# Boese0601/MagicDance

Measured on NVIDIA H100. Metric: denoise-steps/sec @512x512 50-step DDIM, higher is better.
Workload: dtype f16

## Files before the change

### magicdance_b200/csrc/attention.cu

```cuda
#include <stdlib.h>

#include <type_traits>

#include "common.cuh"

namespace mdb {

constexpr int kBQ = 128;

template <int D, int BKV, int STAGES>
struct AttnCfg {
  static constexpr int kDkChunks = (D + 63) / 64;
  static constexpr int kDV = (D + 15) / 16 * 16;
  static constexpr int kKSteps = kDV / 16;
  static constexpr int kQBytes = kDkChunks * kBQ * 128;
  static constexpr int kKBytes = kDkChunks * BKV * 128;
  static constexpr int kVBytes = kDV * 128;
  static constexpr int kStageBytes = kKBytes + kVBytes;
  static constexpr int kSmem = kQBytes + STAGES * kStageBytes + 1024;
  static_assert(BKV == 64, "one 128-byte swizzle row of keys per V^T tile");
  static_assert(kVBytes % 1024 == 0 && kKBytes % 1024 == 0, "stage tiles start on swizzle-atom boundaries");
};

struct AttnKParams {
  CUtensorMap tmQ, tmK0, tmV0, tmK1, tmV1;
  __half* out;
  long long ldo;
  int nq, n0, n1;
  int kv0_batches, kv1_batches;
  int ldv0_batch, ldv1_batch;
  int bank_batches;
  float scale_log2;
};
struct AttnLseKParams : AttnKParams {
  float* lse;
};

template <int D, int BKV, int STAGES, int MINB, bool LSE = false>
__global__ void __launch_bounds__(kWsThreads, MINB)
    attn_wg_kernel(const __grid_constant__ std::conditional_t<LSE, AttnLseKParams, AttnKParams> p) {
  using C = AttnCfg<D, BKV, STAGES>;
  extern __shared__ uint8_t smem_raw[];
  __shared__ __align__(8) uint64_t q_bar;
  __shared__ __align__(8) uint64_t kv_full[STAGES], kv_empty[STAGES];

  uint8_t* sQ = align1024(smem_raw);
  uint8_t* sKV = sQ + C::kQBytes;

  const int warp = threadIdx.x >> 5;
  const int lane = threadIdx.x & 31;
  const int q0 = blockIdx.x * kBQ;
  const int head = blockIdx.y;
  const int b = blockIdx.z;
  const int t0 = (p.n0 + BKV - 1) / BKV;
  const int t1 = (b < p.bank_batches && p.n1 > 0) ? (p.n1 + BKV - 1) / BKV : 0;
  const int n_tiles = t0 + t1;

  pdl_launch_dependents();
  if (warp == kProducerWarp && lane == 0) {
    tma_prefetch_desc(&p.tmQ);
    tma_prefetch_desc(&p.tmK0);
    tma_prefetch_desc(&p.tmV0);
    mbar_init(&q_bar, 1);
    ring_init<STAGES>(kv_full, kv_empty, 1);
    fence_barrier_init();
  }
  __syncthreads();
  pdl_wait();

  if (warp == kProducerWarp) {
    if (lane == 0) {
      mbar_expect_tx(&q_bar, C::kQBytes);
      for (int dc = 0; dc < C::kDkChunks; ++dc)
        tma_load_3d(sQ + dc * (kBQ * 128), &p.tmQ, &q_bar, dc * 64, head, b * p.nq + q0);
      for (int j = 0; j < n_tiles; ++j) {
        const bool src1 = j >= t0;
        const int key0 = (src1 ? (j - t0) : j) * BKV;
        const CUtensorMap* tk = src1 ? &p.tmK1 : &p.tmK0;
        const CUtensorMap* tv = src1 ? &p.tmV1 : &p.tmV0;
        const int nsrc = src1 ? p.n1 : p.n0;
        const int kvb = src1 ? (p.kv1_batches > 1 ? b : 0) : (p.kv0_batches > 1 ? b : 0);
        const int ldvb = src1 ? p.ldv1_batch : p.ldv0_batch;
        const int s = ring_acquire<STAGES>(kv_empty, j);
        mbar_expect_tx(&kv_full[s], C::kStageBytes);
        uint8_t* sk = sKV + s * C::kStageBytes;
        uint8_t* sv = sk + C::kKBytes;
        for (int dc = 0; dc < C::kDkChunks; ++dc)
          tma_load_3d(sk + dc * (BKV * 128), tk, &kv_full[s], dc * 64, head, kvb * nsrc + key0);
        tma_load_2d(sv, tv, &kv_full[s], kvb * ldvb + key0, head * D);
      }
    }
  } else {
    const int wg = warp >> 2;
    const uint32_t q_addr = smem_u32(sQ) + wg * (64 * 128);
    const int cq = 2 * (lane & 3);
    float o[C::kDV / 2];
#pragma unroll
    for (int i = 0; i < C::kDV / 2; ++i) o[i] = 0.f;
    float m_run[2] = {-INFINITY, -INFINITY};
    float l_run[2] = {0.f, 0.f};
    mbar_wait(&q_bar, 0);

    for (int j = 0; j < n_tiles; ++j) {
      const bool src1 = j >= t0;
      const int key0 = (src1 ? (j - t0) : j) * BKV;
      const int valid = min(BKV, (src1 ? p.n1 : p.n0) - key0);
      const int s = ring_wait_full<STAGES>(kv_full, j);
      const uint32_t k_addr = smem_u32(sKV + s * C::kStageBytes);
      const uint32_t v_addr = k_addr + C::kKBytes;

      float sc[BKV / 2];
      wgmma_fence();
#pragma unroll
      for (int ks = 0; ks < C::kKSteps; ++ks) {
        const int dc = ks >> 2, kk = ks & 3;
        const uint64_t da = wgmma_desc_k_sw128(q_addr + dc * (kBQ * 128)) + 2 * kk;
        const uint64_t db = wgmma_desc_k_sw128(k_addr + dc * (BKV * 128)) + 2 * kk;
        wgmma_ss<BKV>(sc, da, db, ks != 0 ? 1u : 0u);
      }
      wgmma_commit();
      wgmma_wait<0>();
      wgmma_fence_regs(sc);

      if (valid < BKV) {
#pragma unroll
        for (int i = 0; i < BKV / 2; ++i)
          if (8 * (i >> 2) + cq + (i & 1) >= valid) sc[i] = -INFINITY;
      }
      float mx[2] = {-INFINITY, -INFINITY};
#pragma unroll
      for (int i = 0; i < BKV / 2; ++i) mx[(i >> 1) & 1] = fmaxf(mx[(i >> 1) & 1], sc[i]);
      float alpha[2], neg_m[2];
#pragma unroll
      for (int h = 0; h < 2; ++h) {
        mx[h] = fmaxf(mx[h], __shfl_xor_sync(0xffffffffu, mx[h], 1));
        mx[h] = fmaxf(mx[h], __shfl_xor_sync(0xffffffffu, mx[h], 2));
        const float m_new = fmaxf(m_run[h], mx[h] * p.scale_log2);
        alpha[h] = ex2_approx(m_run[h] - m_new);
        m_run[h] = m_new;
        neg_m[h] = -m_new;
      }
      float ls[2] = {0.f, 0.f};
      uint32_t pa[BKV / 16][4];
#pragma unroll
      for (int i = 0; i < BKV / 2; i += 2) {
        const int h = (i >> 1) & 1;
        const float e0 = ex2_approx(fmaf(sc[i], p.scale_log2, neg_m[h]));
        const float e1 = ex2_approx(fmaf(sc[i + 1], p.scale_log2, neg_m[h]));
        ls[h] += e0 + e1;
        pa[i >> 3][(i >> 1) & 3] = pack_half2(e0, e1);
      }
#pragma unroll
      for (int h = 0; h < 2; ++h) l_run[h] = fmaf(l_run[h], alpha[h], ls[h]);
#pragma unroll
      for (int i = 0; i < C::kDV / 2; ++i) o[i] *= alpha[(i >> 1) & 1];

      wgmma_fence();
#pragma unroll
      for (int kk = 0; kk < BKV / 16; ++kk)
        wgmma_rs<C::kDV>(o, pa[kk], wgmma_desc_k_sw128(v_addr) + 2 * kk, 1u);
      wgmma_commit();
      wgmma_wait<0>();
      wgmma_fence_regs(o);
      mbar_arrive(&kv_empty[s]);
    }

    float inv_l[2], l_row[2];
#pragma unroll
    for (int h = 0; h < 2; ++h) {
      float l = l_run[h];
      l += __shfl_xor_sync(0xffffffffu, l, 1);
      l += __shfl_xor_sync(0xffffffffu, l, 2);
      inv_l[h] = 1.0f / l;
      l_row[h] = l;
    }
    const int r = wg * 64 + (warp & 3) * 16 + (lane >> 2);
    if constexpr (LSE) {
      if ((lane & 3) == 0) {
#pragma unroll
        for (int h = 0; h < 2; ++h) {
          const int q = q0 + r + 8 * h;
          if (q < p.nq)
            p.lse[(static_cast<long long>(b) * gridDim.y + head) * p.nq + q] =
                (m_run[h] + log2f(l_row[h])) * 0.6931471805599453f;
        }
      }
    }
#pragma unroll
    for (int h = 0; h < 2; ++h) {
      const int q = q0 + r + 8 * h;
      if (q < p.nq) {
        __half* op = p.out + (static_cast<long long>(b) * p.nq + q) * p.ldo + head * D + cq;
#pragma unroll
        for (int c8 = 0; c8 < D / 8; ++c8)
          *reinterpret_cast<uint32_t*>(op + 8 * c8) =
              pack_half2(o[4 * c8 + 2 * h] * inv_l[h], o[4 * c8 + 2 * h + 1] * inv_l[h]);
      }
    }
  }
}

static int g_attn40_2q_min_ctas = 512;
int get_attn_tuning() { return g_attn40_2q_min_ctas; }
void set_attn_tuning(int v) { g_attn40_2q_min_ctas = v; }

template <int D, int BKV, int STAGES, int MINB, bool LSE = false, typename P>
static int launch_attn(const P& kp, dim3 grid, cudaStream_t st) {
  using C = AttnCfg<D, BKV, STAGES>;
  static_assert(MINB == 1 || C::kSmem <= 113 * 1024, "two CTAs per SM must fit");
  constexpr auto kern = attn_wg_kernel<D, BKV, STAGES, MINB, LSE>;
  if (int rc = set_max_dyn_smem<kern>(C::kSmem)) return rc;
  MDB_CHECK_CUDA(launch_pdl(kern, grid, dim3(kWsThreads), C::kSmem, st, kp));
  count_launch();
  return MDB_OK;
}

template <int D, int BKV>
static int build_and_launch(const mdb_attn_desc* a, float* lse, cudaStream_t st) {
  constexpr int kDV = AttnCfg<D, BKV, 1>::kDV;
  AttnKParams kp;
  memset(&kp, 0, sizeof(kp));
  const int hd = a->heads * a->d;
  int rc;
  if ((rc = tmap_heads(&kp.tmQ, a->q, a->d, a->heads, (uint64_t)a->batch * a->nq, a->ldq, kBQ))) return rc;
  auto mk_kv = [&](const void* k, long long ldk, const void* vt, long long ldvt, int n, int nb, int ldvb,
                   CUtensorMap* tk, CUtensorMap* tv) -> int {
    int r = tmap_heads(tk, k, a->d, a->heads, (uint64_t)nb * n, ldk, BKV);
    if (r) return r;
    return tmap_rows(tv, vt, (uint64_t)nb * ldvb, hd, ldvt, 64, kDV);
  };
  if ((rc = mk_kv(a->k0, a->ldk0, a->vt0, a->ldvt0, a->n0, a->kv0_batches, a->ldv0_batch, &kp.tmK0, &kp.tmV0))) return rc;
  if (a->n1 > 0) {
    if ((rc = mk_kv(a->k1, a->ldk1, a->vt1, a->ldvt1, a->n1, a->kv1_batches, a->ldv1_batch, &kp.tmK1, &kp.tmV1)))
      return rc;
  }
  kp.out = static_cast<__half*>(a->out);
  kp.ldo = a->ldo;
  kp.nq = a->nq;
  kp.n0 = a->n0;
  kp.n1 = a->n1;
  kp.kv0_batches = a->kv0_batches;
  kp.kv1_batches = a->kv1_batches;
  kp.ldv0_batch = a->ldv0_batch;
  kp.ldv1_batch = a->ldv1_batch;
  kp.bank_batches = a->n1 > 0 ? a->bank_batches : 0;
  kp.scale_log2 = a->scale * 1.4426950408889634f;
  dim3 grid((a->nq + kBQ - 1) / kBQ, a->heads, a->batch);
  if (lse != nullptr) {
    AttnLseKParams lp;
    memset(&lp, 0, sizeof(lp));
    static_cast<AttnKParams&>(lp) = kp;
    lp.lse = lse;
    if constexpr (D == 40) {
      const long long ctas = (long long)grid.x * grid.y * grid.z;
      if (ctas >= (long long)g_attn40_2q_min_ctas) return launch_attn<D, BKV, 3, 2, true>(lp, grid, st);
    }
    return launch_attn<D, BKV, (D == 160 ? 2 : 4), 1, true>(lp, grid, st);
  }
  if constexpr (D == 40) {
    const long long ctas = (long long)grid.x * grid.y * grid.z;
    if (ctas >= (long long)g_attn40_2q_min_ctas) return launch_attn<D, BKV, 3, 2>(kp, grid, st);
  }
// ... 48 lines not shown
```

### magicdance_b200/csrc/common.cuh

```cuda
#pragma once

#include <cuda.h>
#include <cuda_fp16.h>
#include <cuda_runtime.h>
#include <cudaTypedefs.h>
#include <stdint.h>
#include <stdio.h>
#include <string.h>

#include "../../include/magicdance_b200.h"
#include "wgmma.cuh"

namespace mdb {

void set_error(const char* fmt, ...);

#define MDB_CHECK_CUDA(expr)                                                                     \
  do {                                                                                           \
    cudaError_t _e = (expr);                                                                     \
    if (_e != cudaSuccess) {                                                                     \
      mdb::set_error("%s:%d: %s failed: %s", __FILE__, __LINE__, #expr, cudaGetErrorString(_e)); \
      return MDB_ERR_CUDA;                                                                       \
    }                                                                                            \
  } while (0)

#define MDB_REQUIRE(cond, ...)      \
  do {                              \
    if (!(cond)) {                  \
      mdb::set_error(__VA_ARGS__);  \
      return MDB_ERR_INVALID;       \
    }                               \
  } while (0)

void count_launch(int n = 1);
int get_gemm_tuning(int key);
void set_gemm_tuning(int key, int value);
int get_attn_tuning();
void set_attn_tuning(int v);

constexpr int kNumSms = 132;

int tmap_rows(CUtensorMap* out, const void* base, uint64_t inner, uint64_t rows, long long ld, uint32_t box_inner,
              uint32_t box_rows);
int tmap_heads(CUtensorMap* out, const void* base, int d, int heads, uint64_t tokens, long long ld,
               uint32_t box_tokens);
int tmap_nhwc(CUtensorMap* out, const void* base, int c, int w, int h, int nb, long long ld, const uint32_t box[4],
              int cs);

enum { kBoxOk, kBoxWideRows, kBoxRowsPerTile, kBoxImagesPerTile, kBoxTooLarge };
int pixel_box(int ho, int wo, int cs, int rows, bool fwd, uint32_t box[4]);

#ifdef __CUDACC__

bool pdl_enabled();
template <typename... KArgs, typename... Args>
inline cudaError_t launch_pdl_cluster2(void (*kernel)(KArgs...), dim3 grid, dim3 block, size_t smem,
                                       cudaStream_t stream, unsigned cluster_x, unsigned cluster_z, Args&&... args) {
  cudaLaunchConfig_t cfg;
  memset(&cfg, 0, sizeof(cfg));
  cfg.gridDim = grid;
  cfg.blockDim = block;
  cfg.dynamicSmemBytes = smem;
  cfg.stream = stream;
  cudaLaunchAttribute attr[2];
  int n = 0;
  if (cluster_z > 1 || cluster_x > 1) {
    attr[n].id = cudaLaunchAttributeClusterDimension;
    attr[n].val.clusterDim.x = cluster_x;
    attr[n].val.clusterDim.y = 1;
    attr[n].val.clusterDim.z = cluster_z;
    ++n;
  }
  if (pdl_enabled()) {
    attr[n].id = cudaLaunchAttributeProgrammaticStreamSerialization;
    attr[n].val.programmaticStreamSerializationAllowed = 1;
    ++n;
// ... 44 lines not shown
}
__device__ __forceinline__ void fence_barrier_init() {
  asm volatile("fence.mbarrier_init.release.cluster;" ::: "memory");
}
__device__ __forceinline__ void mbar_expect_tx(uint64_t* bar, uint32_t bytes) {
  asm volatile("mbarrier.arrive.expect_tx.shared::cta.b64 _, [%0], %1;" ::"r"(smem_u32(bar)), "r"(bytes)
               : "memory");
}
__device__ __forceinline__ void mbar_arrive(uint64_t* bar) {
  asm volatile("mbarrier.arrive.shared::cta.b64 _, [%0];" ::"r"(smem_u32(bar)) : "memory");
}
__device__ __forceinline__ void mbar_wait(uint64_t* bar, uint32_t parity) {
  uint32_t addr = smem_u32(bar);
  asm volatile(
      "{\n\t.reg .pred P1;\n\t"
      "WAIT_LOOP:\n\t"
      "mbarrier.try_wait.parity.shared::cta.b64 P1, [%0], %1;\n\t"
      "@P1 bra DONE;\n\t"
      "bra WAIT_LOOP;\n\t"
      "DONE:\n\t}"
      ::"r"(addr), "r"(parity)
      : "memory");
}

constexpr int kConsumers = 256;
constexpr int kProducerWarp = kConsumers / 32;
constexpr int kWsThreads = kConsumers + 32;

__device__ __forceinline__ uint8_t* align1024(uint8_t* p) {
  return reinterpret_cast<uint8_t*>((reinterpret_cast<uintptr_t>(p) + 1023) & ~uintptr_t(1023));
}

template <int S>
__device__ __forceinline__ void ring_init(uint64_t* full, uint64_t* empty, uint32_t full_count) {
  for (int s = 0; s < S; ++s) {
    mbar_init(&full[s], full_count);
    mbar_init(&empty[s], kConsumers);
  }
}
template <int S>
__device__ __forceinline__ int ring_acquire(uint64_t* empty, int it) {
  const int s = it % S;
  mbar_wait(&empty[s], ((it / S) & 1) ^ 1);
  return s;
}
template <int S>
__device__ __forceinline__ int ring_wait_full(uint64_t* full, int it) {
  const int s = it % S;
  mbar_wait(&full[s], (it / S) & 1);
  return s;
}

__device__ __forceinline__ void tma_prefetch_desc(const CUtensorMap* m) {
  asm volatile("prefetch.tensormap [%0];" ::"l"(reinterpret_cast<uint64_t>(m)) : "memory");
}
__device__ __forceinline__ void tma_load_2d(void* dst, const CUtensorMap* m, uint64_t* bar, int c0, int c1) {
  asm volatile(
      "cp.async.bulk.tensor.2d.shared::cluster.global.tile.mbarrier::complete_tx::bytes [%0], [%1, {%3, %4}], [%2];"
      ::"r"(smem_u32(dst)), "l"(reinterpret_cast<uint64_t>(m)), "r"(smem_u32(bar)), "r"(c0), "r"(c1)
      : "memory");
}
__device__ __forceinline__ void tma_load_3d(void* dst, const CUtensorMap* m, uint64_t* bar, int c0, int c1, int c2) {
  asm volatile(
      "cp.async.bulk.tensor.3d.shared::cluster.global.tile.mbarrier::complete_tx::bytes [%0], [%1, {%3, %4, %5}], [%2];"
      ::"r"(smem_u32(dst)), "l"(reinterpret_cast<uint64_t>(m)), "r"(smem_u32(bar)), "r"(c0), "r"(c1), "r"(c2)
      : "memory");
}
__device__ __forceinline__ void tma_load_4d(void* dst, const CUtensorMap* m, uint64_t* bar, int c0, int c1, int c2,
                                            int c3) {
  asm volatile(
// ... 76 lines not shown
```

### magicdance_b200/csrc/gemm.cu

```cuda
#include <stdlib.h>

#include "common.cuh"

namespace mdb {

constexpr int kBM = 128;
constexpr int kBK = 64;

struct GemmKParams {
  CUtensorMap tmA;
  CUtensorMap tmA2;
  CUtensorMap tmB;
  __half* d;
  long long ldd;
  const float* bias;
  long long bias_batch_stride;
  const __half* residual;
  long long ldr;
  float* ws;
  int rows_per_batch;
  int m, n;
  int k_chunks;
  int k1_chunks;
  int chunks_per_split;
  int splits;
  int conv;
  int chunks_per_tap;
  int w, hw;
  int cs;
  int cluster_reduce;
  const float* ln_u;
  float ln_eps;
};

template <int BN, int STAGES>
struct GemmSmem {
  static constexpr int kABytes = kBM * kBK * 2;
  static constexpr int kBBytes = BN * kBK * 2;
  static constexpr int kStageBytes = kABytes + kBBytes;
  static constexpr int kTotal = STAGES * kStageBytes + 1024;
  static constexpr int kCtasPerSm = (kTotal <= 113 * 1024 && BN <= 128) ? 2 : 1;
};

__device__ __forceinline__ void epi_store_chunk(const GemmKParams& p, long long row, int col0, int ncols,
                                                float (&v)[32], const float* bias_chunk) {
  const __half* rp = (p.residual != nullptr) ? p.residual + row * p.ldr + col0 : nullptr;
  __half* dp = p.d + row * p.ldd + col0;
#pragma unroll
  for (int q = 0; q < 4; ++q) {
    if (q * 8 + 8 <= ncols) {
      float o[8];
#pragma unroll
      for (int e = 0; e < 8; ++e) o[e] = v[q * 8 + e];
      if (bias_chunk != nullptr) {
        const float4 b0 = *reinterpret_cast<const float4*>(bias_chunk + q * 8);
        const float4 b1 = *reinterpret_cast<const float4*>(bias_chunk + q * 8 + 4);
        o[0] += b0.x; o[1] += b0.y; o[2] += b0.z; o[3] += b0.w;
        o[4] += b1.x; o[5] += b1.y; o[6] += b1.z; o[7] += b1.w;
      }
      if (rp != nullptr) {
        const uint4 r4 = *reinterpret_cast<const uint4*>(rp + q * 8);
        const __half2* h2 = reinterpret_cast<const __half2*>(&r4);
#pragma unroll
        for (int e = 0; e < 4; ++e) {
          const float2 f = __half22float2(h2[e]);
          o[2 * e] += f.x;
          o[2 * e + 1] += f.y;
        }
      }
      uint4 o4;
      o4.x = pack_half2(o[0], o[1]);
      o4.y = pack_half2(o[2], o[3]);
      o4.z = pack_half2(o[4], o[5]);
      o4.w = pack_half2(o[6], o[7]);
      *reinterpret_cast<uint4*>(dp + q * 8) = o4;
    } else if (q * 8 < ncols) {
// ... 24 lines not shown

  uint8_t* smem = align1024(smem_raw);
  const int warp = threadIdx.x >> 5;
  const int lane = threadIdx.x & 31;
  const int m0 = blockIdx.x * kBM;
  const int n0 = blockIdx.y * BN;
  const int split = blockIdx.z;
  const int kc_begin = split * p.chunks_per_split;
  const int kc_end = min(p.k_chunks, kc_begin + p.chunks_per_split);
  const int n_iter = kc_end - kc_begin;
  constexpr int kRedLd = BN + 4;
  static_assert(kBM * kRedLd * 4 <= kStages * S::kStageBytes, "the accumulator tile must fit in the operand ring");
  const bool ln = p.ln_u != nullptr;

  pdl_launch_dependents();
  if (warp == kProducerWarp && lane == 0) {
    tma_prefetch_desc(&p.tmA);
    tma_prefetch_desc(&p.tmB);
    ring_init<kStages>(full_bar, empty_bar, 1);
    fence_barrier_init();
  }
  const bool bias_in_smem = (p.bias != nullptr) && (p.bias_batch_stride == 0) && !p.cluster_reduce;
  if (bias_in_smem && warp < kProducerWarp) {
    for (int j = threadIdx.x; j < BN; j += kConsumers) s_bias[j] = (n0 + j < p.n) ? p.bias[n0 + j] : 0.f;
  }
  if (ln && warp < kProducerWarp) {
    for (int j = threadIdx.x; j < BN; j += kConsumers) s_lnu[j] = (n0 + j < p.n) ? p.ln_u[n0 + j] : 0.f;
  }
  __syncthreads();
  pdl_wait();

  if (warp == kProducerWarp) {
    if (lane == 0 && n_iter > 0) {
      int b0 = 0, y0 = 0, x0 = 0;
      if (p.conv) {
        b0 = m0 / p.hw;
        y0 = (p.hw >= kBM) ? (m0 % p.hw) / p.w : 0;
        x0 = (p.hw >= kBM) ? (m0 % p.hw) % p.w : 0;
      }
      for (int it = 0; it < n_iter; ++it) {
        const int s = ring_acquire<kStages>(empty_bar, it);
        uint8_t* sa = smem + s * S::kStageBytes;
        uint8_t* sb = sa + S::kABytes;
        const int kc = kc_begin + it;
        mbar_expect_tx(&full_bar[s], S::kStageBytes);
        if (p.conv) {
          const int tap = kc / p.chunks_per_tap;
          const int cc = kc - tap * p.chunks_per_tap;
          const int kh = tap / 3, kw = tap - kh * 3;
          tma_load_4d(sa, &p.tmA, &full_bar[s], cc * kBK, p.cs * x0 + kw - 1, p.cs * y0 + kh - 1, b0);
        } else if (kc < p.k1_chunks) {
          tma_load_2d(sa, &p.tmA, &full_bar[s], kc * kBK, m0);
        } else {
          tma_load_2d(sa, &p.tmA2, &full_bar[s], (kc - p.k1_chunks) * kBK, m0);
        }
        tma_load_2d(sb, &p.tmB, &full_bar[s], kc * kBK, n0);
      }
    }
  } else {
    const int wg = warp >> 2;
    const int tid = threadIdx.x;
    float acc[BN / 2];
#pragma unroll
    for (int i = 0; i < BN / 2; ++i) acc[i] = 0.f;
    const int ln_row = tid >> 1, ln_half = tid & 1;
    float pivot = 0.f, ls0 = 0.f, ls1 = 0.f, lq0 = 0.f, lq1 = 0.f;
    for (int it = 0; it < n_iter; ++it) {
      const int s = ring_wait_full<kStages>(full_bar, it);
      const uint32_t a_addr = smem_u32(smem + s * S::kStageBytes);
      const uint64_t da = wgmma_desc_k_sw128(a_addr + wg * (64 * 128));
      const uint64_t db = wgmma_desc_k_sw128(a_addr + S::kABytes);
      wgmma_fence();
#pragma unroll
      for (int k = 0; k < kBK / 16; ++k) wgmma_ss<BN>(acc, da + 2 * k, db + 2 * k, 1u);
      wgmma_commit();
      if (ln) {
        const uint32_t arow = a_addr + (ln_row >> 3) * 1024 + (ln_row & 7) * 128;
        if (it == 0) {
          uint32_t w0;
          asm volatile("ld.shared.b32 %0, [%1];" : "=r"(w0) : "r"(arow + ((0 ^ (ln_row & 7)) << 4)));
          pivot = __low2float(*reinterpret_cast<const __half2*>(&w0));
        }
#pragma unroll
        for (int l = ln_half * 4; l < ln_half * 4 + 4; ++l) {
          uint4 u4;
          asm volatile("ld.shared.v4.b32 {%0, %1, %2, %3}, [%4];"
                       : "=r"(u4.x), "=r"(u4.y), "=r"(u4.z), "=r"(u4.w)
                       : "r"(arow + ((l ^ (ln_row & 7)) << 4)));
          const __half2* h2 = reinterpret_cast<const __half2*>(&u4);
// ... 227 lines not shown
      }
      if (p.bias != nullptr) {
        const long long brow = (p.bias_batch_stride != 0) ? (row / p.rows_per_batch) : 0;
        const float* bp = p.bias + brow * p.bias_batch_stride + col;
        a.x += bp[0]; a.y += bp[1]; a.z += bp[2]; a.w += bp[3];
      }
      if (p.residual != nullptr) {
        const __half2* rp = reinterpret_cast<const __half2*>(p.residual + row * p.ldr + col);
        const float2 r0 = __half22float2(rp[0]), r1 = __half22float2(rp[1]);
        a.x += r0.x; a.y += r0.y; a.z += r1.x; a.w += r1.y;
      }
      uint2 o;
      o.x = pack_half2(a.x, a.y);
      o.y = pack_half2(a.z, a.w);
      *reinterpret_cast<uint2*>(p.d + row * p.ldd + col) = o;
    }
    return;
  }
  for (long long i = static_cast<long long>(blockIdx.x) * blockDim.x + threadIdx.x; i < slab;
       i += static_cast<long long>(gridDim.x) * blockDim.x) {
    const long long row = i / p.n;
    const int col = static_cast<int>(i - row * p.n);
    float v = 0.f;
    for (int s = 0; s < p.splits; ++s) v += p.ws[s * slab + i];
    if (p.bias != nullptr) {
      const long long brow = (p.bias_batch_stride != 0) ? (row / p.rows_per_batch) : 0;
      v += p.bias[brow * p.bias_batch_stride + col];
    }
    if (p.residual != nullptr) v += __half2float(p.residual[row * p.ldr + col]);
    p.d[row * p.ldd + col] = __float2half_rn(v);
  }
}

int pixel_box(int ho, int wo, int cs, int rows, bool fwd, uint32_t box[4]) {
  const int hw = ho * wo;
  if (fwd ? wo > rows : wo >= rows) {
    if (wo % rows || (fwd && cs != 1)) return kBoxWideRows;
    box[1] = cs * rows; box[2] = 1; box[3] = 1;
  } else if (hw >= rows) {
    if (rows % wo || hw % rows) return kBoxRowsPerTile;
    box[1] = cs * wo; box[2] = cs * (rows / wo); box[3] = 1;
  } else {
    if (rows % hw) return kBoxImagesPerTile;
    box[1] = cs * wo; box[2] = cs * ho; box[3] = rows / hw;
  }
  box[0] = 64;
  return box[1] <= 256 && box[2] <= 256 ? kBoxOk : kBoxTooLarge;
}

static int g_pair_min_tiles = 128;
static int g_bn80_below = 100;
constexpr int kLongKChunks = 64;

template <int BN, bool GEGLU, int STAGES>
static int launch_gemm(const GemmKParams& kp, dim3 grid, cudaStream_t st) {
  const unsigned cluster_z = kp.cluster_reduce ? static_cast<unsigned>(kp.splits) : 1u;
  constexpr auto kern = gemm_tc_kernel<BN, GEGLU, STAGES>;
  constexpr int kSmem = GemmSmem<BN, STAGES>::kTotal;
  static_assert(kSmem <= 227 * 1024, "shared memory budget");
  if (int rc = set_max_dyn_smem<kern>(kSmem)) return rc;
  MDB_CHECK_CUDA(launch_pdl_cluster(kern, grid, dim3(kWsThreads), kSmem, st, cluster_z, kp));
  count_launch();
  return MDB_OK;
}

int get_gemm_tuning(int key) { return key == MDB_TUNE_GEMM_PAIR_MIN_TILES ? g_pair_min_tiles : g_bn80_below; }
void set_gemm_tuning(int key, int value) {
  if (key == MDB_TUNE_GEMM_PAIR_MIN_TILES) g_pair_min_tiles = value;
  else g_bn80_below = value;
}

}

using namespace mdb;

extern "C" int mdb_gemm_f16(const mdb_gemm_desc* g, mdb_stream_t stream) {
  MDB_REQUIRE(g != nullptr, "mdb_gemm_f16: null descriptor");
  MDB_REQUIRE(g->m > 0 && g->n > 0 && g->k > 0, "mdb_gemm_f16: bad shape m=%d n=%d k=%d", g->m, g->n, g->k);
  MDB_REQUIRE(g->k % kBK == 0, "mdb_gemm_f16: K=%d must be a multiple of 64", g->k);
  MDB_REQUIRE(g->a && g->b && g->d, "mdb_gemm_f16: null operand");
  cudaStream_t st = static_cast<cudaStream_t>(stream);
  const bool geglu = g->epilogue == MDB_EPI_GEGLU;
  GemmKParams kp;
  memset(&kp, 0, sizeof(kp));
  kp.d = static_cast<__half*>(g->d);
  kp.ldd = g->ldd;
  kp.bias = g->bias;
  kp.bias_batch_stride = g->bias_batch_stride;
  kp.rows_per_batch = g->rows_per_batch > 0 ? g->rows_per_batch : 1;
  kp.residual = static_cast<const __half*>(g->residual);
  kp.ldr = g->ldr;
  kp.m = g->m;
  kp.n = g->n;
  kp.k_chunks = g->k / kBK;
// ... 72 lines not shown
    const bool wide_split = g->splits == 0 && kp.k_chunks >= kLongKChunks && tiles160 * 2 <= kNumSms;
    bn = (tiles160 < g_bn80_below && !wide_split) ? 80 : 160;
  } else {
    bn = 128;
  }
  rc = tmap_rows(&kp.tmB, g->b, g->k, g->n, g->ldb, kBK, bn);
  if (rc) return rc;

  int splits = g->splits > 1 ? g->splits : 1;
  if (g->ln_u != nullptr) splits = 1;
  if (g->splits == 0 && !geglu && !pair && g->ln_u == nullptr) {
    const long long tiles = (long long)m_tiles * ((g->n + bn - 1) / bn);
    if (tiles < 100)
      for (int c = 8; c >= 2; c >>= 1)
        if (tiles * c <= kNumSms && kp.k_chunks / c >= 16) {
          splits = c;
          break;
        }
  }
  if (splits > kp.k_chunks) splits = kp.k_chunks;
  if (geglu || pair) splits = 1;
  kp.chunks_per_split = (kp.k_chunks + splits - 1) / splits;
  splits = (kp.k_chunks + kp.chunks_per_split - 1) / kp.chunks_per_split;
  kp.splits = splits;
  kp.ws = g->splitk_ws;
  kp.cluster_reduce = (!geglu && (splits == 2 || splits == 4 || splits == 8)) ? 1 : 0;
  if (splits > 1 && !kp.cluster_reduce) {
    MDB_REQUIRE(g->splitk_ws != nullptr, "mdb_gemm_f16: splits > 1 needs splitk_ws");
  }

  dim3 grid(m_tiles, (g->n + bn - 1) / bn, splits);
  const bool deep = (long long)grid.x * grid.y * grid.z <= kNumSms && kp.chunks_per_split >= 12;
  if (pair) {
    if (bn == 256) rc = geglu ? launch_gemm<256, true, 4>(kp, grid, st) : launch_gemm<256, false, 4>(kp, grid, st);
    else if (bn == 160) rc = launch_gemm<160, false, 6>(kp, grid, st);
    else rc = launch_gemm<128, false, 6>(kp, grid, st);
    return rc;
  }
  if (geglu) rc = launch_gemm<128, true, 3>(kp, grid, st);
  else if (bn == 160) rc = deep ? launch_gemm<160, false, 6>(kp, grid, st) : launch_gemm<160, false, 3>(kp, grid, st);
  else if (bn == 80) rc = deep ? launch_gemm<80, false, 8>(kp, grid, st) : launch_gemm<80, false, 3>(kp, grid, st);
  else rc = deep ? launch_gemm<128, false, 6>(kp, grid, st) : launch_gemm<128, false, 3>(kp, grid, st);
  if (rc) return rc;
  if (splits > 1 && !kp.cluster_reduce) {
    const long long total = ((long long)g->m * g->n + 3) / 4;
    int blocks = (int)((total + 255) / 256);
    if (blocks > kNumSms * 8) blocks = kNumSms * 8;
    MDB_CHECK_CUDA(launch_pdl(splitk_finalize_kernel, dim3(blocks), dim3(256), 0, st, kp));
    count_launch();
  }
  return MDB_OK;
}
```

### magicdance_b200/csrc/misc.cu

```cuda
#include <stdarg.h>
#include <stdlib.h>

#include <atomic>

#include "common.cuh"

namespace mdb {

static thread_local char g_err[512] = "";
static std::atomic<long long> g_launches{0};

void set_error(const char* fmt, ...) {
  va_list ap;
  va_start(ap, fmt);
  vsnprintf(g_err, sizeof(g_err), fmt, ap);
  va_end(ap);
}
void count_launch(int n) { g_launches.fetch_add(n, std::memory_order_relaxed); }
bool pdl_enabled() { return true; }

static PFN_cuTensorMapEncodeTiled_v12000 g_encode = nullptr;

static int make_tmap_f16(CUtensorMap* out, const void* base, int rank, const uint64_t* dims,
                         const uint64_t* strides_bytes, const uint32_t* box, const uint32_t* elem_strides = nullptr) {
  if (g_encode == nullptr) {
    void* fn = nullptr;
    cudaDriverEntryPointQueryResult qres;
    cudaError_t e = cudaGetDriverEntryPoint("cuTensorMapEncodeTiled", &fn, cudaEnableDefault, &qres);
    if (e != cudaSuccess || fn == nullptr || qres != cudaDriverEntryPointSuccess) {
      set_error("cuTensorMapEncodeTiled not available from the driver (%s)", cudaGetErrorString(e));
      return MDB_ERR_CUDA;
    }
    g_encode = reinterpret_cast<PFN_cuTensorMapEncodeTiled_v12000>(fn);
  }
  cuuint64_t gdim[5];
  cuuint64_t gstr[4];
  cuuint32_t bx[5];
  cuuint32_t es[5];
  for (int i = 0; i < rank; ++i) {
    gdim[i] = dims[i];
    bx[i] = box[i];
    es[i] = elem_strides ? elem_strides[i] : 1;
    if (i > 0) gstr[i - 1] = strides_bytes[i - 1];
  }
  if ((reinterpret_cast<uintptr_t>(base) & 15) != 0) {
    set_error("TMA base address %p is not 16-byte aligned", base);
    return MDB_ERR_INVALID;
  }
  for (int i = 0; i + 1 < rank; ++i) {
    if (gstr[i] % 16 != 0) {
      set_error("TMA stride %d (%llu bytes) is not a multiple of 16", i, (unsigned long long)gstr[i]);
      return MDB_ERR_INVALID;
    }
  }
  CUresult r = g_encode(out, CU_TENSOR_MAP_DATA_TYPE_FLOAT16, rank, const_cast<void*>(base), gdim, gstr, bx, es,
                        CU_TENSOR_MAP_INTERLEAVE_NONE, CU_TENSOR_MAP_SWIZZLE_128B, CU_TENSOR_MAP_L2_PROMOTION_L2_256B,
                        CU_TENSOR_MAP_FLOAT_OOB_FILL_NONE);
  if (r != CUDA_SUCCESS) {
    set_error("cuTensorMapEncodeTiled failed with CUresult %d (rank %d, dims %llu,%llu box %u,%u)", (int)r, rank,
              (unsigned long long)gdim[0], (unsigned long long)(rank > 1 ? gdim[1] : 0), bx[0], rank > 1 ? bx[1] : 0);
    return MDB_ERR_CUDA;
  }
  return MDB_OK;
}

int tmap_rows(CUtensorMap* out, const void* base, uint64_t inner, uint64_t rows, long long ld, uint32_t box_inner,
              uint32_t box_rows) {
  const uint64_t dims[2] = {inner, rows};
  const uint64_t str[1] = {(uint64_t)ld * 2};
  const uint32_t box[2] = {box_inner, box_rows};
  return make_tmap_f16(out, base, 2, dims, str, box);
}

int tmap_heads(CUtensorMap* out, const void* base, int d, int heads, uint64_t tokens, long long ld,
               uint32_t box_tokens) {
  const uint64_t dims[3] = {(uint64_t)d, (uint64_t)heads, tokens};
  const uint64_t str[2] = {(uint64_t)d * 2, (uint64_t)ld * 2};
  const uint32_t box[3] = {64, 1, box_tokens};
  return make_tmap_f16(out, base, 3, dims, str, box);
}

int tmap_nhwc(CUtensorMap* out, const void* base, int c, int w, int h, int nb, long long ld, const uint32_t box[4],
              int cs) {
  const uint64_t dims[4] = {(uint64_t)c, (uint64_t)w, (uint64_t)h, (uint64_t)nb};
  const uint64_t str[3] = {(uint64_t)ld * 2, (uint64_t)ld * w * 2, (uint64_t)ld * h * w * 2};
  const uint32_t estr[4] = {1u, (uint32_t)cs, (uint32_t)cs, 1u};
  return make_tmap_f16(out, base, 4, dims, str, box, cs == 2 ? estr : nullptr);
}

constexpr int kDcTile = 8;
constexpr int kDcCout = 32;
constexpr int kDcCin = 16;

template <int STRIDE>
__global__ void __launch_bounds__(256) direct_conv3x3_kernel(const __half* __restrict__ x, const __half* __restrict__ wt,
                                                             const float* __restrict__ bias,
                                                             const __half* __restrict__ residual, __half* __restrict__ y,
                                                             int h, int w, int cin, int cout, int ho, int wo, int silu) {
  constexpr int PH = (kDcTile - 1) * STRIDE + 3;
  pdl_launch_dependents();
  pdl_wait();
  __shared__ float s_in[PH * PH * kDcCin];
  __shared__ float s_w[kDcCout * 9 * kDcCin];
  const int tiles_x = (wo + kDcTile - 1) / kDcTile;
// ... 681 lines not shown
```

Before: 89.93.

## Overlap next QK^T wgmma with PV and compute row sums via padded ones column

Software-pipelines the attention loop so the next tile's QK^T wgmma is issued right after the PV wgmma, deferring the wait and the stage release by one iteration when only one CTA runs per SM. For head dims that are padded (kDV > D), the padding rows of V^T are filled with half-precision ones so the PV MMA also produces the softmax denominator, removing the scalar row-sum accumulation. The V TMA now loads only D rows, and the tuning threshold for the two-Q variant is halved. This trades register pressure and a deeper in-flight wgmma chain for less serialization.

```diff
diff --git a/magicdance_b200/csrc/attention.cu b/magicdance_b200/csrc/attention.cu
--- a/magicdance_b200/csrc/attention.cu
+++ b/magicdance_b200/csrc/attention.cu
@@ -17,6 +17,8 @@
   static constexpr int kKBytes = kDkChunks * BKV * 128;
   static constexpr int kVBytes = kDV * 128;
   static constexpr int kStageBytes = kKBytes + kVBytes;
+  static constexpr bool kSumByMma = kDV > D;
+  static constexpr int kStageTxBytes = kKBytes + D * 128;
   static constexpr int kSmem = kQBytes + STAGES * kStageBytes + 1024;
   static_assert(BKV == 64, "one 128-byte swizzle row of keys per V^T tile");
   static_assert(kVBytes % 1024 == 0 && kKBytes % 1024 == 0, "stage tiles start on swizzle-atom boundaries");
@@ -64,6 +66,12 @@
     mbar_init(&q_bar, 1);
     ring_init<STAGES>(kv_full, kv_empty, 1);
     fence_barrier_init();
+  }
+  if constexpr (C::kSumByMma) {
+    constexpr int kWords = (C::kDV - D) * 128 / 4;
+    for (int i = threadIdx.x; i < STAGES * kWords; i += blockDim.x)
+      reinterpret_cast<uint32_t*>(sKV + (i / kWords) * C::kStageBytes + C::kKBytes + D * 128)[i % kWords] = 0x3c003c00u;
+    fence_proxy_async_smem();
   }
   __syncthreads();
   pdl_wait();
@@ -82,7 +90,7 @@
         const int kvb = src1 ? (p.kv1_batches > 1 ? b : 0) : (p.kv0_batches > 1 ? b : 0);
         const int ldvb = src1 ? p.ldv1_batch : p.ldv0_batch;
         const int s = ring_acquire<STAGES>(kv_empty, j);
-        mbar_expect_tx(&kv_full[s], C::kStageBytes);
+        mbar_expect_tx(&kv_full[s], C::kStageTxBytes);
         uint8_t* sk = sKV + s * C::kStageBytes;
         uint8_t* sv = sk + C::kKBytes;
         for (int dc = 0; dc < C::kDkChunks; ++dc)
@@ -99,17 +107,9 @@
     for (int i = 0; i < C::kDV / 2; ++i) o[i] = 0.f;
     float m_run[2] = {-INFINITY, -INFINITY};
     float l_run[2] = {0.f, 0.f};
-    mbar_wait(&q_bar, 0);
-
-    for (int j = 0; j < n_tiles; ++j) {
-      const bool src1 = j >= t0;
-      const int key0 = (src1 ? (j - t0) : j) * BKV;
-      const int valid = min(BKV, (src1 ? p.n1 : p.n0) - key0);
-      const int s = ring_wait_full<STAGES>(kv_full, j);
-      const uint32_t k_addr = smem_u32(sKV + s * C::kStageBytes);
-      const uint32_t v_addr = k_addr + C::kKBytes;
-
-      float sc[BKV / 2];
+    float sc[BKV / 2];
+    auto issue_qk = [&](int jj) {
+      const uint32_t k_addr = smem_u32(sKV + ring_wait_full<STAGES>(kv_full, jj) * C::kStageBytes);
       wgmma_fence();
 #pragma unroll
       for (int ks = 0; ks < C::kKSteps; ++ks) {
@@ -119,8 +119,24 @@
         wgmma_ss<BKV>(sc, da, db, ks != 0 ? 1u : 0u);
       }
       wgmma_commit();
+    };
+    mbar_wait(&q_bar, 0);
+    constexpr bool kOverlap = MINB == 1 && D != 160;
+    wgmma_fence_regs(o);
+    if constexpr (kOverlap) issue_qk(0);
+
+    for (int j = 0; j < n_tiles; ++j) {
+      const bool src1 = j >= t0;
+      const int key0 = (src1 ? (j - t0) : j) * BKV;
+      const int valid = min(BKV, (src1 ? p.n1 : p.n0) - key0);
+      const int s = j % STAGES;
+      const uint32_t v_addr = smem_u32(sKV + s * C::kStageBytes) + C::kKBytes;
+
+      if constexpr (!kOverlap) issue_qk(j);
       wgmma_wait<0>();
       wgmma_fence_regs(sc);
+      wgmma_fence_regs(o);
+      if (kOverlap && j > 0) mbar_arrive(&kv_empty[(j - 1) % STAGES]);
 
       if (valid < BKV) {
 #pragma unroll
@@ -147,11 +163,12 @@
         const int h = (i >> 1) & 1;
         const float e0 = ex2_approx(fmaf(sc[i], p.scale_log2, neg_m[h]));
         const float e1 = ex2_approx(fmaf(sc[i + 1], p.scale_log2, neg_m[h]));
-        ls[h] += e0 + e1;
+        if constexpr (!C::kSumByMma) ls[h] += e0 + e1;
         pa[i >> 3][(i >> 1) & 3] = pack_half2(e0, e1);
       }
 #pragma unroll
-      for (int h = 0; h < 2; ++h) l_run[h] = fmaf(l_run[h], alpha[h], ls[h]);
+      for (int h = 0; h < 2; ++h)
+        if constexpr (!C::kSumByMma) l_run[h] = fmaf(l_run[h], alpha[h], ls[h]);
 #pragma unroll
       for (int i = 0; i < C::kDV / 2; ++i) o[i] *= alpha[(i >> 1) & 1];
 
@@ -160,17 +177,28 @@
       for (int kk = 0; kk < BKV / 16; ++kk)
         wgmma_rs<C::kDV>(o, pa[kk], wgmma_desc_k_sw128(v_addr) + 2 * kk, 1u);
       wgmma_commit();
-      wgmma_wait<0>();
-      wgmma_fence_regs(o);
-      mbar_arrive(&kv_empty[s]);
-    }
+      if constexpr (kOverlap) {
+        if (j + 1 < n_tiles) issue_qk(j + 1);
+      } else {
+        wgmma_wait<0>();
+        wgmma_fence_regs(o);
+        mbar_arrive(&kv_empty[s]);
+      }
+    }
+    wgmma_wait<0>();
+    wgmma_fence_regs(o);
 
     float inv_l[2], l_row[2];
 #pragma unroll
     for (int h = 0; h < 2; ++h) {
-      float l = l_run[h];
-      l += __shfl_xor_sync(0xffffffffu, l, 1);
-      l += __shfl_xor_sync(0xffffffffu, l, 2);
+      float l;
+      if constexpr (C::kSumByMma) {
+        l = __shfl_sync(0xffffffffu, o[4 * (D / 8) + 2 * h], lane & ~3);
+      } else {
+        l = l_run[h];
+        l += __shfl_xor_sync(0xffffffffu, l, 1);
+        l += __shfl_xor_sync(0xffffffffu, l, 2);
+      }
       inv_l[h] = 1.0f / l;
       l_row[h] = l;
     }
@@ -200,7 +228,7 @@
   }
 }
 
-static int g_attn40_2q_min_ctas = 512;
+static int g_attn40_2q_min_ctas = 256;
 int get_attn_tuning() { return g_attn40_2q_min_ctas; }
 void set_attn_tuning(int v) { g_attn40_2q_min_ctas = v; }
 
@@ -217,7 +245,6 @@
 
 template <int D, int BKV>
 static int build_and_launch(const mdb_attn_desc* a, float* lse, cudaStream_t st) {
-  constexpr int kDV = AttnCfg<D, BKV, 1>::kDV;
   AttnKParams kp;
   memset(&kp, 0, sizeof(kp));
   const int hd = a->heads * a->d;
@@ -227,7 +254,7 @@
                    CUtensorMap* tk, CUtensorMap* tv) -> int {
     int r = tmap_heads(tk, k, a->d, a->heads, (uint64_t)nb * n, ldk, BKV);
     if (r) return r;
-    return tmap_rows(tv, vt, (uint64_t)nb * ldvb, hd, ldvt, 64, kDV);
+    return tmap_rows(tv, vt, (uint64_t)nb * ldvb, hd, ldvt, 64, D);
   };
   if ((rc = mk_kv(a->k0, a->ldk0, a->vt0, a->ldvt0, a->n0, a->kv0_batches, a->ldv0_batch, &kp.tmK0, &kp.tmV0))) return rc;
   if (a->n1 > 0) {
```

New measurement: 90.72 (median of 6 runs). No clear change (+0.9%).

## Add persistent ping-pong WGMMA GEMM for large BN=160 paired launches

Applied to the files above, without the earlier changes.

Adds a persistent GEMM kernel with one TMA producer warp and two consumer warpgroups. The consumers alternate tiles, so one warpgroup's epilogue overlaps the other's K-loop, and register counts are rebalanced with setmaxnreg. The residual tile is prefetched by TMA through a new non-swizzled tensor map, and output goes through a shared-memory staging buffer for coalesced 16-byte stores. It is used only for BN=160 paired GEMMs with at least two waves of tiles, replacing the 6-stage non-persistent kernel with a 4-stage pipeline, which risks less latency hiding per tile.

```diff
diff --git a/magicdance_b200/csrc/common.cuh b/magicdance_b200/csrc/common.cuh
--- a/magicdance_b200/csrc/common.cuh
+++ b/magicdance_b200/csrc/common.cuh
@@ -41,7 +41,7 @@
 constexpr int kNumSms = 132;
 
 int tmap_rows(CUtensorMap* out, const void* base, uint64_t inner, uint64_t rows, long long ld, uint32_t box_inner,
-              uint32_t box_rows);
+              uint32_t box_rows, bool swizzle = true);
 int tmap_heads(CUtensorMap* out, const void* base, int d, int heads, uint64_t tokens, long long ld,
                uint32_t box_tokens);
 int tmap_nhwc(CUtensorMap* out, const void* base, int c, int w, int h, int nb, long long ld, const uint32_t box[4],
@@ -152,10 +152,11 @@
 }
 
 template <int S>
-__device__ __forceinline__ void ring_init(uint64_t* full, uint64_t* empty, uint32_t full_count) {
+__device__ __forceinline__ void ring_init(uint64_t* full, uint64_t* empty, uint32_t full_count,
+                                          uint32_t empty_count = kConsumers) {
   for (int s = 0; s < S; ++s) {
     mbar_init(&full[s], full_count);
-    mbar_init(&empty[s], kConsumers);
+    mbar_init(&empty[s], empty_count);
   }
 }
 template <int S>
diff --git a/magicdance_b200/csrc/gemm.cu b/magicdance_b200/csrc/gemm.cu
--- a/magicdance_b200/csrc/gemm.cu
+++ b/magicdance_b200/csrc/gemm.cu
@@ -11,6 +11,7 @@
   CUtensorMap tmA;
   CUtensorMap tmA2;
   CUtensorMap tmB;
+  CUtensorMap tmR;
   __half* d;
   long long ldd;
   const float* bias;
@@ -42,6 +43,31 @@
   static constexpr int kCtasPerSm = (kTotal <= 113 * 1024 && BN <= 128) ? 2 : 1;
 };
 
+struct TileLoader {
+  int m0, n0;
+  int b0 = 0, y0 = 0, x0 = 0;
+  __device__ __forceinline__ TileLoader(const GemmKParams& p, int m0_, int n0_) : m0(m0_), n0(n0_) {
+    if (p.conv) {
+      b0 = m0 / p.hw;
+      y0 = (p.hw >= kBM) ? (m0 % p.hw) / p.w : 0;
+      x0 = (p.hw >= kBM) ? (m0 % p.hw) % p.w : 0;
+    }
+  }
+  __device__ __forceinline__ void load(const GemmKParams& p, uint8_t* sa, int a_bytes, uint64_t* bar, int kc) const {
+    if (p.conv) {
+      const int tap = kc / p.chunks_per_tap;
+      const int cc = kc - tap * p.chunks_per_tap;
+      const int kh = tap / 3, kw = tap - kh * 3;
+      tma_load_4d(sa, &p.tmA, bar, cc * kBK, p.cs * x0 + kw - 1, p.cs * y0 + kh - 1, b0);
+    } else if (kc < p.k1_chunks) {
+      tma_load_2d(sa, &p.tmA, bar, kc * kBK, m0);
+    } else {
+      tma_load_2d(sa, &p.tmA2, bar, (kc - p.k1_chunks) * kBK, m0);
+    }
+    tma_load_2d(sa + a_bytes, &p.tmB, bar, kc * kBK, n0);
+  }
+};
+
 __device__ __forceinline__ void epi_store_chunk(const GemmKParams& p, long long row, int col0, int ncols,
                                                 float (&v)[32], const float* bias_chunk) {
   const __half* rp = (p.residual != nullptr) ? p.residual + row * p.ldr + col0 : nullptr;
@@ -132,29 +158,11 @@
 
   if (warp == kProducerWarp) {
     if (lane == 0 && n_iter > 0) {
-      int b0 = 0, y0 = 0, x0 = 0;
-      if (p.conv) {
-        b0 = m0 / p.hw;
-        y0 = (p.hw >= kBM) ? (m0 % p.hw) / p.w : 0;
-        x0 = (p.hw >= kBM) ? (m0 % p.hw) % p.w : 0;
-      }
+      const TileLoader ld(p, m0, n0);
       for (int it = 0; it < n_iter; ++it) {
         const int s = ring_acquire<kStages>(empty_bar, it);
-        uint8_t* sa = smem + s * S::kStageBytes;
-        uint8_t* sb = sa + S::kABytes;
-        const int kc = kc_begin + it;
         mbar_expect_tx(&full_bar[s], S::kStageBytes);
-        if (p.conv) {
-          const int tap = kc / p.chunks_per_tap;
-          const int cc = kc - tap * p.chunks_per_tap;
-          const int kh = tap / 3, kw = tap - kh * 3;
-          tma_load_4d(sa, &p.tmA, &full_bar[s], cc * kBK, p.cs * x0 + kw - 1, p.cs * y0 + kh - 1, b0);
-        } else if (kc < p.k1_chunks) {
-          tma_load_2d(sa, &p.tmA, &full_bar[s], kc * kBK, m0);
-        } else {
-          tma_load_2d(sa, &p.tmA2, &full_bar[s], (kc - p.k1_chunks) * kBK, m0);
-        }
-        tma_load_2d(sb, &p.tmB, &full_bar[s], kc * kBK, n0);
+        ld.load(p, smem + s * S::kStageBytes, S::kABytes, &full_bar[s], kc_begin + it);
       }
     }
   } else {
@@ -448,6 +456,157 @@
   }
 }
 
+template <int BN, int STAGES>
+struct PersistentSmem {
+  static constexpr int kABytes = kBM * kBK * 2;
+  static constexpr int kBBytes = BN * kBK * 2;
+  static constexpr int kStageBytes = kABytes + kBBytes;
+  static constexpr int kOutBytes = kBM * BN * 2;
+  static constexpr int kTotal = STAGES * kStageBytes + 2 * kOutBytes + 1024;
+};
+
+constexpr int kPersistentThreads = kConsumers + 128;
+
+template <int BN, int STAGES>
+__global__ void __launch_bounds__(kPersistentThreads, 1) gemm_persistent_kernel(const __grid_constant__ GemmKParams p) {
+  using S = PersistentSmem<BN, STAGES>;
+  extern __shared__ uint8_t smem_raw[];
+  __shared__ __align__(8) uint64_t full_bar[STAGES];
+  __shared__ __align__(8) uint64_t empty_bar[STAGES];
+  __shared__ __align__(8) uint64_t kloop_bar[2];
+  __shared__ __align__(8) uint64_t res_bar[2];
+
+  uint8_t* smem = align1024(smem_raw);
+  const int warp = threadIdx.x >> 5;
+  const int lane = threadIdx.x & 31;
+  const int n_tiles = (p.n + BN - 1) / BN;
+  const int tiles = ((p.m + kBM - 1) / kBM) * n_tiles;
+  const int kcn = p.k_chunks;
+  constexpr int kWgThreads = kConsumers / 2;
+
+  pdl_launch_dependents();
+  if (warp == kProducerWarp && lane == 0) {
+    tma_prefetch_desc(&p.tmA);
+    tma_prefetch_desc(&p.tmB);
+    ring_init<STAGES>(full_bar, empty_bar, 1, kWgThreads);
+    mbar_init(&kloop_bar[0], kWgThreads);
+    mbar_init(&kloop_bar[1], kWgThreads);
+    mbar_init(&res_bar[0], 1);
+    mbar_init(&res_bar[1], 1);
+    fence_barrier_init();
+  }
+  __syncthreads();
+  pdl_wait();
+
+  if (warp >= kProducerWarp) {
+    asm volatile("setmaxnreg.dec.sync.aligned.u32 40;\n");
+    if (warp == kProducerWarp && lane == 0) {
+      int g = 0;
+      for (int t = blockIdx.x; t < tiles; t += gridDim.x) {
+        const TileLoader ld(p, (t / n_tiles) * kBM, (t % n_tiles) * BN);
+        for (int kc = 0; kc < kcn; ++kc, ++g) {
+          const int s = ring_acquire<STAGES>(empty_bar, g);
+          mbar_expect_tx(&full_bar[s], S::kStageBytes);
+          ld.load(p, smem + s * S::kStageBytes, S::kABytes, &full_bar[s], kc);
+        }
+      }
+    }
+    return;
+  }
+
+  asm volatile("setmaxnreg.inc.sync.aligned.u32 232;\n");
+  const int wg = warp >> 2;
+  const int wtid = threadIdx.x & (kWgThreads - 1);
+  __half* tile_buf = reinterpret_cast<__half*>(smem + STAGES * S::kStageBytes + wg * S::kOutBytes);
+  const bool residual = p.residual != nullptr;
+  float acc[2][BN / 2];
+  int i = wg;
+  for (int t = blockIdx.x + wg * gridDim.x; t < tiles; t += 2 * gridDim.x, i += 2) {
+    const int m0 = (t / n_tiles) * kBM;
+    const int n0 = (t % n_tiles) * BN;
+    const int g0 = i * kcn;
+    if (residual) {
+      named_bar_sync(2 + wg, kWgThreads);
+      if (wtid == 0) {
+        mbar_expect_tx(&res_bar[wg], S::kOutBytes);
+        tma_load_2d(tile_buf, &p.tmR, &res_bar[wg], n0, m0);
+      }
+    }
+#pragma unroll
+    for (int j = 0; j < BN / 2; ++j) acc[0][j] = acc[1][j] = 0.f;
+    if (i > 0) mbar_wait(&kloop_bar[wg ^ 1], ((i - 1) >> 1) & 1);
+    for (int kc = 0; kc < kcn; ++kc) {
+      const int s = ring_wait_full<STAGES>(full_bar, g0 + kc);
+      const uint32_t a_addr = smem_u32(smem + s * S::kStageBytes);
+      const uint64_t da0 = wgmma_desc_k_sw128(a_addr);
+      const uint64_t da1 = wgmma_desc_k_sw128(a_addr + 64 * 128);
+      const uint64_t db = wgmma_desc_k_sw128(a_addr + S::kABytes);
+      wgmma_fence();
+#pragma unroll
+      for (int k = 0; k < kBK / 16; ++k) {
+        wgmma_ss<BN>(acc[0], da0 + 2 * k, db + 2 * k, 1u);
+        wgmma_ss<BN>(acc[1], da1 + 2 * k, db + 2 * k, 1u);
+      }
+      wgmma_commit();
+      wgmma_wait<1>();
+      wgmma_fence_regs(acc[0]);
+      wgmma_fence_regs(acc[1]);
+      if (kc > 0) mbar_arrive(&empty_bar[(g0 + kc - 1) % STAGES]);
+    }
+    mbar_arrive(&kloop_bar[wg]);
+    wgmma_wait<0>();
+    wgmma_fence_regs(acc[0]);
+    wgmma_fence_regs(acc[1]);
+    mbar_arrive(&empty_bar[(g0 + kcn - 1) % STAGES]);
+
+    if (residual) mbar_wait(&res_bar[wg], (i >> 1) & 1);
+    const int r_base = (warp & 3) * 16 + (lane >> 2);
+#pragma unroll
+    for (int h = 0; h < 2; ++h) {
+#pragma unroll
+      for (int rh = 0; rh < 2; ++rh) {
+        const int rl = h * 64 + r_base + 8 * rh;
+        const int row = m0 + rl;
+        const bool row_ok = row < p.m;
+        const long long brow = (p.bias_batch_stride != 0 && row_ok) ? (row / p.rows_per_batch) : 0;
+        const float* bias_row = (p.bias != nullptr) ? p.bias + brow * p.bias_batch_stride : nullptr;
+#pragma unroll
+        for (int j = 2 * rh; j < BN / 2; j += 4) {
+          const int cl = 8 * (j >> 2) + 2 * (lane & 3);
+          const int col = n0 + cl;
+          __half2* t = reinterpret_cast<__half2*>(tile_buf + rl * BN + cl);
+          float o0 = acc[h][j], o1 = acc[h][j + 1];
+          if (row_ok && col < p.n) {
+            if (bias_row != nullptr) {
+              const float2 b = *reinterpret_cast<const float2*>(bias_row + col);
+              o0 += b.x;
+              o1 += b.y;
+            }
+            if (residual) {
+              const float2 f = __half22float2(*t);
+              o0 += f.x;
+              o1 += f.y;
+            }
+          }
+          *reinterpret_cast<uint32_t*>(t) = pack_half2(o0, o1);
+        }
+      }
+    }
+    named_bar_sync(2 + wg, kWgThreads);
+    constexpr int kRowChunks = BN / 8;
+#pragma unroll 4
+    for (int q = wtid; q < kBM * kRowChunks; q += kWgThreads) {
+      const int r = q / kRowChunks, c = q - r * kRowChunks;
+      const long long row = static_cast<long long>(m0) + r;
+      const int col = n0 + c * 8;
+      if (row < p.m && col < p.n)
+        *reinterpret_cast<uint4*>(p.d + row * p.ldd + col) = *reinterpret_cast<const uint4*>(tile_buf + r * BN + c * 8);
+    }
+    fence_proxy_async_smem();
+    if (!residual) named_bar_sync(2 + wg, kWgThreads);
+  }
+}
+
 int pixel_box(int ho, int wo, int cs, int rows, bool fwd, uint32_t box[4]) {
   const int hw = ho * wo;
   if (fwd ? wo > rows : wo >= rows) {
@@ -476,6 +635,18 @@
   static_assert(kSmem <= 227 * 1024, "shared memory budget");
   if (int rc = set_max_dyn_smem<kern>(kSmem)) return rc;
   MDB_CHECK_CUDA(launch_pdl_cluster(kern, grid, dim3(kWsThreads), kSmem, st, cluster_z, kp));
+  count_launch();
+  return MDB_OK;
+}
+
+template <int BN, int STAGES>
+static int launch_gemm_persistent(const GemmKParams& kp, long long tiles, cudaStream_t st) {
+  constexpr auto kern = gemm_persistent_kernel<BN, STAGES>;
+  constexpr int kSmem = PersistentSmem<BN, STAGES>::kTotal;
+  static_assert(kSmem + 1024 <= 227 * 1024, "shared memory budget (dynamic + the kernel's barriers)");
+  if (int rc = set_max_dyn_smem<kern>(kSmem)) return rc;
+  const dim3 grid(static_cast<unsigned>(tiles < kNumSms ? tiles : kNumSms));
+  MDB_CHECK_CUDA(launch_pdl(kern, grid, dim3(kPersistentThreads), kSmem, st, kp));
   count_launch();
   return MDB_OK;
 }
@@ -614,6 +785,14 @@
   dim3 grid(m_tiles, (g->n + bn - 1) / bn, splits);
   const bool deep = (long long)grid.x * grid.y * grid.z <= kNumSms && kp.chunks_per_split >= 12;
   if (pair) {
+    const long long tiles = (long long)grid.x * grid.y;
+    if (bn == 160 && tiles >= 2 * kNumSms) {
+      if (g->residual) {
+        rc = tmap_rows(&kp.tmR, g->residual, g->n, g->m, g->ldr, 160, kBM, false);
+        if (rc) return rc;
+      }
+      return launch_gemm_persistent<160, 4>(kp, tiles, st);
+    }
     if (bn == 256) rc = geglu ? launch_gemm<256, true, 4>(kp, grid, st) : launch_gemm<256, false, 4>(kp, grid, st);
     else if (bn == 160) rc = launch_gemm<160, false, 6>(kp, grid, st);
     else rc = launch_gemm<128, false, 6>(kp, grid, st);
diff --git a/magicdance_b200/csrc/misc.cu b/magicdance_b200/csrc/misc.cu
--- a/magicdance_b200/csrc/misc.cu
+++ b/magicdance_b200/csrc/misc.cu
@@ -22,7 +22,8 @@
 static PFN_cuTensorMapEncodeTiled_v12000 g_encode = nullptr;
 
 static int make_tmap_f16(CUtensorMap* out, const void* base, int rank, const uint64_t* dims,
-                         const uint64_t* strides_bytes, const uint32_t* box, const uint32_t* elem_strides = nullptr) {
+                         const uint64_t* strides_bytes, const uint32_t* box, const uint32_t* elem_strides = nullptr,
+                         bool swizzle = true) {
   if (g_encode == nullptr) {
     void* fn = nullptr;
     cudaDriverEntryPointQueryResult qres;
@@ -54,7 +55,8 @@
     }
   }
   CUresult r = g_encode(out, CU_TENSOR_MAP_DATA_TYPE_FLOAT16, rank, const_cast<void*>(base), gdim, gstr, bx, es,
-                        CU_TENSOR_MAP_INTERLEAVE_NONE, CU_TENSOR_MAP_SWIZZLE_128B, CU_TENSOR_MAP_L2_PROMOTION_L2_256B,
+                        CU_TENSOR_MAP_INTERLEAVE_NONE, swizzle ? CU_TENSOR_MAP_SWIZZLE_128B : CU_TENSOR_MAP_SWIZZLE_NONE,
+                        CU_TENSOR_MAP_L2_PROMOTION_L2_256B,
                         CU_TENSOR_MAP_FLOAT_OOB_FILL_NONE);
   if (r != CUDA_SUCCESS) {
     set_error("cuTensorMapEncodeTiled failed with CUresult %d (rank %d, dims %llu,%llu box %u,%u)", (int)r, rank,
@@ -65,11 +67,11 @@
 }
 
 int tmap_rows(CUtensorMap* out, const void* base, uint64_t inner, uint64_t rows, long long ld, uint32_t box_inner,
-              uint32_t box_rows) {
+              uint32_t box_rows, bool swizzle) {
   const uint64_t dims[2] = {inner, rows};
   const uint64_t str[1] = {(uint64_t)ld * 2};
   const uint32_t box[2] = {box_inner, box_rows};
-  return make_tmap_f16(out, base, 2, dims, str, box);
+  return make_tmap_f16(out, base, 2, dims, str, box, nullptr, swizzle);
 }
 
 int tmap_heads(CUtensorMap* out, const void* base, int d, int heads, uint64_t tokens, long long ld,
```

Result: faster. 90.23 before, 91.82 after (median of 6 runs) (+1.8%).
